# teboli/polyblur

Hardware: AMD Instinct MI355X
Metric: megapixels/sec (n_iter=3, alpha=6, beta=1) (higher is better)
Workload: dtype f32; 1 GPU; batch=1 3840x2160x3 fp32 per GPU, n_iter=3, method=fft (circular), full 25-tap support; mode=resident, images_per_gpu=1, height=2160, width=3840, parallelism=images sharded, no data-path collective

## Files before the change

polyblur_amd/csrc/api.hip:

```cpp
#include <algorithm>
#include <cstdlib>
#include <cstring>

#include "common.h"

int pb_grad_energy(pb_ctx *ctx, const void *gx, const void *gy, float *nM, int P, long HW, int g_dtype = PB_F32);
int pb_halo_apply(pb_ctx *ctx, const void *x, int x_dtype, int x_pitch, long x_plane, const float *y, const void *gx,
                  const void *gy, const void *ox, const float *nM, void *out, int out_dtype, int P, int H, int W,
                  int clamp01, const void *recomb_cur = nullptr, int recomb_cur_dtype = 0, const float *recomb_smooth = nullptr,
                  int g_dtype = PB_F32);
int pb_recombine(pb_ctx *ctx, const float *y, const void *cur, int cur_dtype, const float *smooth, void *out, int out_dtype,
                 long n);
int pb_bilateral5_impl(pb_ctx *ctx, const void *in, int in_dtype, void *out, int out_dtype, int P, int H, int W);
int pb_dt_filter_impl(pb_ctx *ctx, const void *in, const void *joint, int dtype, float *out, int B, int C, int H, int W,
                      float sigma_s, float sigma_r, int num_iterations);
int pb_nc_filter_impl(pb_ctx *ctx, const void *in, int dtype, float *out, int B, int C, int H, int W, float sigma_s,
                      float sigma_r, int num_iterations);
int pb_convert_from_float(pb_ctx *ctx, const float *in, void *out, int dtype, long n);
int pb_u8_layout(pb_ctx *ctx, const unsigned char *in, unsigned char *out, int B, int C, int H, int W, int to_planar);
int pb_convert_to_float(pb_ctx *ctx, const void *in, int dtype, float *out, long n);
int pb_extract_patches_impl(pb_ctx *ctx, const void *img, void *patches, int dtype, int B, int C, int H, int W, int ph, int pw,
                            int step_h, int step_w, int n_j, int pad_top, int pad_left, int first, int count);
int pb_overlap_add_impl(pb_ctx *ctx, const void *patches, void *out, int dtype, int B, int C, int H, int W, int ph, int pw,
                        int step_h, int step_w, int n_i, int n_j, int pad_top, int pad_left, const float *win_y,
// ... 32 lines not shown
    return b.p;
}

static size_t dsize(int dtype) { return dtype == PB_F16 ? 2 : (dtype == PB_U8 ? 1 : 4); }
static int pitch4(int w) { return (w + 3) & ~3; }

static void pb_read_knobs(pb_ctx *ctx) {
    auto geti = [](const char *n, int &v) { if (const char *e = getenv(n)) v = atoi(e); };
    auto getl = [](const char *n, long &v) { if (const char *e = getenv(n)) v = atol(e); };
    if (const char *e = getenv("PB_FFT_BODY")) ctx->fft_wave = (e[0] == 'w' && e[1] == 'g') ? 0 : 1;
#ifdef PB_EXPERIMENTAL
    geti("PB_STRIP", ctx->strip_mode);
#endif
    geti("PB_EST_GRAY_ROWS", ctx->est_gray_rows); geti("PB_EST_LEAN", ctx->est_lean); geti("PB_DT_ROWS_REG", ctx->dt_rows_reg); geti("PB_DT_COLS_STRIP", ctx->dt_cols_strip); geti("PB_DT_COLS_COOP", ctx->dt_cols_coop);
    geti("PB_FFT_EXT_RADIX", ctx->fft_ext_radix); geti("PB_FFT_FIRST", ctx->fft_first); geti("PB_FFT_FIRST_ROWS", ctx->fft_first_rows); geti("PB_COLS_FIXED", ctx->cols_fixed); geti("PB_ROWS_FIXED", ctx->rows_fixed);
    geti("PB_POLY1", ctx->poly_mode);
    geti("PB_POLY_ALWAYS", ctx->poly_always); geti("PB_POLY_PADDED", ctx->poly_padded); geti("PB_TAPER_RING", ctx->taper_ring); geti("PB_ZERO_RING", ctx->zero_ring); getl("PB_ZERO_RING_MIN_PAIRS", ctx->zero_ring_min_pairs);
}

extern "C" {

int pb_version(void) { return PB_VERSION; }

void pb_default_options(pb_options *o) {
    memset(o, 0, sizeof(*o));
    o->n_iter = 1; o->c = 0.352f; o->b = 0.768f; o->alpha = 2.f; o->beta = 3.f;
    o->sigma_r = 0.8f; o->sigma_s = 2.0f; o->q = 0.f; o->n_angles = 6; o->n_interpolated_angles = 30;
    o->remove_halo = 0; o->edgetaping = 0; o->prefilter = PB_PREFILTER_NONE; o->discard_saturation = 0;
    o->boundary = PB_WRAP; o->support = PB_SUPPORT_FULL; o->force_theta_deg = -1.f; o->ker_size = PB_KSIZE;
}

// ... 229 lines not shown
    steps[2] = p;
}

PolySpec poly_spec(pb_ctx *ctx, const ConvPass *steps, float alpha, float beta, bool gaussians) {
    const int mode = pb_poly_spec_mode(ctx, steps);
    if (!mode) {
        if (steps[0].boundary == PB_ZERO && gaussians && ctx->poly_always && pb_poly_three_steps_ok(ctx, steps)) {
            PolySpec ps = no_poly();
            ps.always = 2;
            return ps;
        }
        return no_poly();
    }
    const int always = (mode == 3 && gaussians && ctx->poly_always) ? 1 : 0;
    if (steps[0].boundary != PB_WRAP && !always) return no_poly();
    return PolySpec{mode, alpha / 2 - beta + 2, 3 * beta - alpha - 6, 5 - 3 * beta + alpha / 2, beta, PB_POLY_GAIN, PB_POLY_MIN_AREA, PB_POLY_COST128, always};
}

int run_polynomial(pb_ctx *ctx, const Geometry &g, const void *xsrc, int x_dtype, const float *xpadded,
                   const pb_blur_info *info, float alpha, float beta, int boundary, float *t1, float *t2, void *dst,
                   int dst_dtype, int clamp01) {
    const float a3 = alpha / 2 - beta + 2, a2 = 3 * beta - alpha - 6, a1 = 5 - 3 * beta + alpha / 2;
    if (g.sep1) {
        const float scale[3] = {a3, 1.f, 1.f}, coef[3] = {a2, a1, beta};
        float *tmp[2] = {t1, t2};
        ConvPass p1 = base_pass(g, g.sep1, boundary), p2 = base_pass(g, g.sep2, boundary);
        set_x_virtual(p1, g, xsrc, x_dtype); set_out_padded(p1, g, g.sep_u);
        set_x_virtual(p2, g, xsrc, x_dtype);
        for (int step = 0; step < 3; ++step) {
            if (step < 2) set_out_padded(p2, g, tmp[step]); else set_out_interior(p2, g, dst, dst_dtype);
            p2.scale = scale[step]; p2.coef = coef[step]; p2.clamp01 = step == 2 ? clamp01 : 0;
// ... 858 lines not shown
```

polyblur_amd/csrc/common.h:

```cpp
#pragma once
#include <hip/hip_runtime.h>
#include <hip/hip_fp16.h>

#include <cstdarg>
#include <cstdio>
#include <map>
#include <string>
#include <vector>

#include "../../include/polyblur_hip.h"


struct FftPlan {
    int n = 0;
    int nstage = 0;
    int radix[24];
    int bluestein_m = 0;
    float2 *tw = nullptr;
    float *drev = nullptr;
    float2 *chirp = nullptr;
    float2 *bfilt_rev = nullptr;
    float *dnat = nullptr;
};

struct ScratchBuf {
    void *p = nullptr;
    size_t bytes = 0;
};

struct ProfRec {
    hipEvent_t a, b;
    int tag;
};

struct PolySpec { int on; float a3, a2, a1, b; float gain; int min_area; float cost128; int always; };
inline PolySpec no_poly() { return PolySpec{0, 0.f, 0.f, 0.f, 0.f, 0.f, 0, 0.f, 0}; }
inline bool same_spec(const PolySpec &x, const PolySpec &y) {
    return x.on == y.on && x.always == y.always &&
           (!x.on || (x.a3 == y.a3 && x.a2 == y.a2 && x.a1 == y.a1 && x.b == y.b && (x.cost128 > 0.f) == (y.cost128 > 0.f)));
}

struct pb_fft_sel { int use_fft; int rf; int strip; int poly; int hx; int hy; int pad_[2]; };

struct SpectraSet {
    bool holds(const void *info, int B) const { return owner && owner == info && n == B; }
    bool holds(const void *info, int B, const PolySpec &s) const { return holds(info, B) && same_spec(built, s); }
    void claim(const void *info, int B, const PolySpec &s, int sel_slot, bool by_estimate) {
        owner = info; n = B; built = s; slot_ = sel_slot; est = by_estimate;
    }
    void drop() { owner = nullptr; n = 0; est = false; }
    void drop_if_overlaps(const void *lo, const void *hi) {
        const char *o = static_cast<const char *>(owner);
        if (o && o < static_cast<const char *>(hi) && static_cast<const char *>(lo) < o + sizeof(pb_blur_info) * (size_t)n) drop();
    }
// ... 45 lines not shown
    int zero_ring = 1;
    int taper_ring = 1;
    int poly_padded = 1;
    int est_lean = 1;
    int dt_cols_strip = 1;
    int dt_cols_coop = 1;
    int dt_rows_reg = 1;
    int poly_always = 1;
    int est_gray_rows = 1;
    int fft_ext_radix = 1;
    int fft_first_rows = -1;
    int fft_first = -1;
    int cols_fixed = 1;
    int rows_fixed = 1;
    size_t phase_budget = 0;
    int strip_mode = 0;
};

int pb_fail(pb_ctx *ctx, int code, const char *fmt, ...);

struct ProfScope {
    pb_ctx *ctx;
    int idx = -1;
    ProfScope(pb_ctx *c, int tag) : ctx(c) {
        if (!c->prof_on) return;
        ProfRec r;
        r.tag = tag;
        hipEvent_t *ev[2] = {&r.a, &r.b};
        for (auto e : ev) {
            if (!c->evpool.empty()) { *e = c->evpool.back(); c->evpool.pop_back(); }
// ... 28 lines not shown
    } while (0)

enum { SRC_VIRTUAL = 0,
       SRC_PADDED = 1 };
enum { OUT_INTERIOR = 0,
       OUT_PADDED = 1 };
enum { EPI_HORNER = 0,
       EPI_TAPER = 1 };

constexpr int PB_SEL_SLOTS = 16;
constexpr int PB_KHAT_STRIDE = 128 * 128;
constexpr int PB_POLY128_MIN_T = 56;
constexpr int PB_POLY_MIN_TX = 24, PB_POLY_MIN_TY = 16;
constexpr float PB_POLY_GAIN = 0.7f;
constexpr int PB_POLY_MIN_AREA = 768;
constexpr float PB_POLY_COST128 = 8.0f;


struct ConvPass {
    const void *in;  int in_kind;  int in_dtype;  int in_pitch;  long in_plane;
    const void *x;   int x_kind;   int x_dtype;   int x_pitch;   long x_plane;
    void *out;       int out_kind; int out_dtype; int out_pitch; long out_plane;
    int H, W;
    int pad;
    int C;
    int P;
    const pb_blur_info *info;
    float scale, coef;
    int boundary;
    int epilogue;
// ... 87 lines not shown
```

polyblur_amd/csrc/conv_wave_common.h:

```cpp
#pragma once
#include "conv_fft_common.h"

namespace {

constexpr int WF_ROWS = 32;
constexpr size_t kWfLdsWave = sizeof(float2) * WF_ROWS * FT_P;

static __device__ const float kC64[64] = {
    1.0f, 0.9951847195625305f, 0.9807852506637573f, 0.9569403529167175f, 0.9238795042037964f, 0.8819212913513184f,
    0.8314695954322815f, 0.7730104327201843f, 0.7071067690849304f, 0.6343932747840881f, 0.5555702447891235f,
    0.4713967442512512f, 0.3826834261417389f, 0.290284663438797f, 0.19509032368659973f, 0.0980171412229538f, 0.0f,
    -0.0980171412229538f, -0.19509032368659973f, -0.290284663438797f, -0.3826834261417389f, -0.4713967442512512f,
    -0.5555702447891235f, -0.6343932747840881f, -0.7071067690849304f, -0.7730104327201843f, -0.8314695954322815f,
    -0.8819212913513184f, -0.9238795042037964f, -0.9569403529167175f, -0.9807852506637573f, -0.9951847195625305f, -1.0f,
    -0.9951847195625305f, -0.9807852506637573f, -0.9569403529167175f, -0.9238795042037964f, -0.8819212913513184f,
    -0.8314695954322815f, -0.7730104327201843f, -0.7071067690849304f, -0.6343932747840881f, -0.5555702447891235f,
    -0.4713967442512512f, -0.3826834261417389f, -0.290284663438797f, -0.19509032368659973f, -0.0980171412229538f, 0.0f,
    0.0980171412229538f, 0.19509032368659973f, 0.290284663438797f, 0.3826834261417389f, 0.4713967442512512f,
    0.5555702447891235f, 0.6343932747840881f, 0.7071067690849304f, 0.7730104327201843f, 0.8314695954322815f,
    0.8819212913513184f, 0.9238795042037964f, 0.9569403529167175f, 0.9807852506637573f, 0.9951847195625305f};
static __device__ const float kS64[64] = {
    0.0f, 0.0980171412229538f, 0.19509032368659973f, 0.290284663438797f, 0.3826834261417389f, 0.4713967442512512f,
    0.5555702447891235f, 0.6343932747840881f, 0.7071067690849304f, 0.7730104327201843f, 0.8314695954322815f,
    0.8819212913513184f, 0.9238795042037964f, 0.9569403529167175f, 0.9807852506637573f, 0.9951847195625305f, 1.0f,
// ... 74 lines not shown
#define PB_S(i) fwd_stage1<i>(v);
    PB_EACH8(PB_S)
#undef PB_S
}
__device__ __forceinline__ void fft64_inv_stage1(cf (&v)[64]) {
#define PB_S(i) inv_stage1<i>(v);
    PB_EACH8(PB_S)
#undef PB_S
}
__device__ __forceinline__ void fft64_inv_stage2(cf (&v)[64]) {
#define PB_S(i) inv_stage2<i>(v);
    PB_EACH8(PB_S)
#undef PB_S
}

__device__ __forceinline__ void swap_halves(cf &hi_part, cf &lo_part) {
    typedef unsigned u2 __attribute__((ext_vector_type(2)));
    const u2 x = __builtin_amdgcn_permlane32_swap(__float_as_uint(hi_part.x), __float_as_uint(lo_part.x), false, false);
    const u2 y = __builtin_amdgcn_permlane32_swap(__float_as_uint(hi_part.y), __float_as_uint(lo_part.y), false, false);
    hi_part = (cf){__uint_as_float(x[0]), __uint_as_float(y[0])};
    lo_part = (cf){__uint_as_float(x[1]), __uint_as_float(y[1])};
}

__device__ __forceinline__ void transpose64(cf (&v)[64], float2 *Z, int lane) {
#pragma unroll
    for (int r = 0; r < 32; ++r) swap_halves(v[r], v[32 + r]);
    const float2 *rd = Z + (lane & 31) * FT_P + (lane & 32);
#pragma unroll
    for (int h = 0; h < 2; ++h) {
#pragma unroll
// ... 81 lines not shown
```

polyblur_amd/csrc/conv_wfft.hip:

```cpp

#include <algorithm>
#include <cstdlib>
#include <type_traits>

#include "conv_wave_common.h"

namespace {

struct WGeom { int ow, oh; };
struct WJobs { int pairs_x, njobs, per; float inv_pairs_x; };
__device__ __forceinline__ int div_rcp(int n, float rcp_d) { return (int)(((float)n + 0.5f) * rcp_d); }
__device__ __forceinline__ WJobs jobs_of(const WGeom &g, int hx, int hy) {
    const int Tx = FT_N - 2 * hx, Ty = FT_N - 2 * hy;
    const int tiles_x = div_rcp(g.ow + Tx - 1, __builtin_amdgcn_rcpf((float)Tx)), tiles_y = div_rcp(g.oh + Ty - 1, __builtin_amdgcn_rcpf((float)Ty));
    WJobs j;
    j.pairs_x = (tiles_x + 1) >> 1;
    j.njobs = j.pairs_x * tiles_y;
    j.per = (j.njobs + 7) >> 3;
    j.inv_pairs_x = __builtin_amdgcn_rcpf((float)j.pairs_x);
    return j;
}

#ifdef PB_WF_TRACE
constexpr int kTraceWaves = 8192, kTraceStamps = 14;
__device__ unsigned long long g_wf_trace[kTraceWaves * kTraceStamps];
#define PB_T(i) do { if (tr) { __builtin_amdgcn_sched_barrier(0); tr[i] = __builtin_readcyclecounter(); __builtin_amdgcn_sched_barrier(0); } } while (0)
#define PB_TWAIT() asm volatile("s_waitcnt vmcnt(0) lgkmcnt(0)" ::: "memory")
#define PB_TRT(i) do { if (tr) tr[i] = __builtin_amdgcn_s_memrealtime(); } while (0)
#else
#define PB_T(i)
#define PB_TWAIT()
// ... 425 lines not shown
    typedef std::integral_constant<int, 6> I6; typedef std::integral_constant<int, 7> I7;
    request(I0{}); request(I1{}); request(I2{}); request(I3{});
    fft64_inv_stage2(v);
    PB_T(8);
    finish(I0{}); request(I4{});
    finish(I1{}); request(I5{});
    finish(I2{}); request(I6{});
    finish(I3{}); request(I7{});
    finish(I4{}); finish(I5{}); finish(I6{}); finish(I7{});
    PB_T(9);
    PB_TWAIT();
    PB_T(10);
    PB_TRT(13);
}

template <typename TIn, typename TX, typename TOut>
__device__ __forceinline__ bool pair_is_fast(const ConvPass &a, int ty, int pxi, int hx, int hy) {
    if (sizeof(TIn) < 2 || a.epilogue != EPI_HORNER) return false;
    if (sizeof(TIn) == 2 && (a.in_pitch & 7) != 0) return false;
    const int Tx = FT_N - 2 * hx, Ty = FT_N - 2 * hy;
    const OutRegion rg = out_region(a);
    const int Hp = a.H + 2 * a.pad, Wp = a.W + 2 * a.pad;
    const int oy0 = rg.y_lo + ty * Ty, wy0 = oy0 - hy, wxA = rg.x_lo + 2 * pxi * Tx - hx, wxB = wxA + Tx;
    const int lo = a.in_kind == SRC_VIRTUAL ? a.pad : 0;
    const bool virt = a.x_kind == SRC_VIRTUAL;
    const int oo = a.out_kind == OUT_INTERIOR ? a.pad : 0, xsh = virt ? a.pad : 0;
    const int xw = virt ? a.W : Wp, xh = virt ? a.H : Hp;
    const int oxA = wxA + hx;
    return wy0 >= lo && wy0 + FT_N <= Hp - lo && wxA >= lo && wxB + FT_N <= Wp - lo && oy0 + Ty <= rg.y_hi && oxA + 2 * Tx <= rg.x_hi &&
           oy0 - xsh >= 0 && oxA - xsh >= 0 && oy0 + Ty - xsh <= xh && oxA + 2 * Tx - xsh <= xw &&
// ... 62 lines not shown

template <typename TIn, typename TX, typename TOut, bool ZERO>
__global__ __launch_bounds__(64, 2) void conv_wfft_kernel(const ConvPass a, const WGeom g) {
    extern __shared__ __attribute__((aligned(16))) char zb[];
    const int lane = threadIdx.x & 63;
    unsigned long long *tr = nullptr;
#ifdef PB_WF_TRACE
    if (blockIdx.x < kTraceWaves) tr = g_wf_trace + (long)blockIdx.x * kTraceStamps;
    PB_T(0);
    PB_TRT(12);
#endif
    const int C = a.C, B = a.P / C;
    const int q = (int)(blockIdx.x & 7u);
    int rem = (int)(blockIdx.x >> 3);
    int img = 0, hx = 0, hy = 0;
    bool fold = false;
    if (B == 1) {
        const PB_CONSTANT pb_fft_sel *s0 = as_constant(a.fsel);
        if (!s0->use_fft || s0->poly == 2 || !poly_match(a.poly, s0->poly)) return;
        hx = s0->hx; hy = s0->hy;
        fold = a.poly == 2 && s0->poly != 0;
    } else {
        auto share_of = [&](int i) -> int {
            if (i >= B) return 0;
            const pb_fft_sel s = a.fsel[i];
            if (!s.use_fft || s.poly == 2 || !poly_match(a.poly, s.poly)) return 0;
            return jobs_of(g, s.hx, s.hy).per * C;
        };
        bool work = false;
        int base = 0;
        for (int c0 = 0; c0 < B; c0 += 64) {
            const int n = share_of(c0 + lane), incl = wave_scan(n, lane);
            const unsigned long long m = __ballot(base + incl > rem);
            if (m) {
                const int l = __builtin_ctzll(m);
                img = c0 + l;
                rem -= base + (__builtin_amdgcn_readlane(incl, l) - __builtin_amdgcn_readlane(n, l));
                work = true;
                break;
            }
            base += __builtin_amdgcn_readlane(incl, 63);
        }
        if (!work) return;
        img = __builtin_amdgcn_readfirstlane(img); rem = __builtin_amdgcn_readfirstlane(rem);
        hx = as_constant(a.fsel + img)->hx; hy = as_constant(a.fsel + img)->hy;
        fold = a.poly == 2 && as_constant(a.fsel + img)->poly != 0;
    }
    const WJobs j = jobs_of(g, hx, hy);
    const int pl = __builtin_amdgcn_readfirstlane(div_rcp(rem, __builtin_amdgcn_rcpf((float)j.per)));
    if (pl >= C) return;
    const int pair = q * j.per + (rem - pl * j.per);
    if (pair >= j.njobs) return;
    const int ty = __builtin_amdgcn_readfirstlane(div_rcp(pair, j.inv_pairs_x)), pxi = pair - ty * j.pairs_x;
    const int plane = img * C + pl;
    const float *kp = a.khat + (long)img * PB_KHAT_STRIDE;
    const pb_blur_info *info = a.info + img;
    if (a.ring && !ring_live(a, ty, pxi, hx, hy)) return;
    const ConvPass af = fold_pass(a, fold);
    if (taper_is_copy(af, ty, pxi, hx, hy)) { copy_pair<TX, TOut>(af, plane, ty, pxi, hx, hy); return; }
    if (pair_is_fast<TIn, TX, TOut>(af, ty, pxi, hx, hy)) wave_pair<1, TIn, TX, TOut, ZERO>(af, info, plane, ty, pxi, hx, hy, zb, kp, tr);
    else if (pair_is_gen<TIn, TX, TOut>(af, pxi, hx)) wave_pair<2, TIn, TX, TOut, ZERO>(af, info, plane, ty, pxi, hx, hy, zb, kp, tr);
    else wave_pair<0, TIn, TX, TOut, ZERO>(af, info, plane, ty, pxi, hx, hy, zb, kp, tr);
}

bool wfft_geometry(const ConvPass &p, bool poly2, float min_area, WGeom &g, long &per_max) {
    g.oh = (p.out_kind == OUT_INTERIOR) ? p.H : p.H + 2 * p.pad;
    g.ow = (p.out_kind == OUT_INTERIOR) ? p.W : p.W + 2 * p.pad;
    per_max = 0;
    for (int hx = 4; hx <= 28; hx += 4) {
        for (int hy = 2; hy <= 30; hy += 2) {
            const int tx = FT_N - 2 * hx, ty = FT_N - 2 * hy;
            const bool three = hx <= 12 && hy <= 12;
            const bool one = poly2 && tx >= PB_POLY_MIN_TX && ty >= PB_POLY_MIN_TY && (float)(tx * ty) >= min_area;
            if (!three && !one) continue;
            const long nj = (long)(((g.ow + tx - 1) / tx + 1) / 2) * ((g.oh + ty - 1) / ty);
            if (nj > (1L << 20)) return false;
            per_max = std::max(per_max, (nj + 7) / 8);
        }
    }
    const long total = 8 * per_max * p.P;
    return total > 0 && total <= (1L << 23);
}

template <typename TIn, typename TX, typename TOut>
int launch_wfft_typed(pb_ctx *ctx, const ConvPass &p, const WGeom &g, long groups) {
    if (p.boundary == PB_ZERO)
        hipLaunchKernelGGL((conv_wfft_kernel<TIn, TX, TOut, true>), dim3((unsigned)groups), dim3(64), kWfLdsWave, ctx->stream, p, g);
    else
        hipLaunchKernelGGL((conv_wfft_kernel<TIn, TX, TOut, false>), dim3((unsigned)groups), dim3(64), kWfLdsWave, ctx->stream, p, g);
    PB_LAUNCH_CHECK();
    return PB_OK;
}

// ... 1 lines not shown

#ifdef PB_WF_TRACE
extern "C" int pb_debug_wf_trace_clear(void) {
    void *p = nullptr;
    if (hipGetSymbolAddress(&p, HIP_SYMBOL(g_wf_trace)) != hipSuccess) return -1;
    return (int)hipMemset(p, 0, sizeof(unsigned long long) * kTraceStamps * kTraceWaves);
}
extern "C" int pb_debug_wf_trace(unsigned long long *host, int n_waves) {
    if (n_waves > kTraceWaves) n_waves = kTraceWaves;
    return (int)hipMemcpyFromSymbol(host, HIP_SYMBOL(g_wf_trace), sizeof(unsigned long long) * kTraceStamps * n_waves);
}
#endif

bool pb_conv_wfft_feasible(const ConvPass &p, bool poly2) {
    WGeom g; long per_max = 0;
    return wfft_geometry(p, poly2, (float)PB_POLY_MIN_AREA, g, per_max);
}

bool pb_conv_wfft_types(const ConvPass &p) {
    switch (p.in_dtype * 9 + p.x_dtype * 3 + p.out_dtype) {
        case 0: case 1: case 3: case 4: case 12: case 13: case 24: case 26: case 6: case 8: case 2: return true;
        default: return false;
    }
}

int pb_launch_conv_wfft(pb_ctx *ctx, const ConvPass &p) {
    if (!pb_conv_wfft_types(p)) return PB_ERR_UNSUPPORTED;
    const bool poly2 = p.poly != 0 && pb_spec_of_spectra(ctx, p.khat).on >= 2;
    const float min_area = (float)PB_POLY_MIN_AREA;
    WGeom g;
    long per_max = 0;
    if (!wfft_geometry(p, poly2, min_area, g, per_max)) {
        if (poly2) return pb_fail(ctx, PB_ERR_UNSUPPORTED, "conv pass: too many windows for the tile-spectrum body");
        return PB_ERR_UNSUPPORTED;
    }
    long groups = 8L * per_max * p.P;
    if (ctx->known_sel) {
        const int B = p.P / p.C;
        long per_sum = 0, jobs = 0;
        for (int b = 0; b < B && b < (int)ctx->known_sel->size(); ++b) {
            const pb_fft_sel &e = (*ctx->known_sel)[(size_t)b];
            const bool takes = e.use_fft && e.poly != 2 && (p.poly == 2 || (e.poly != 0) == (p.poly != 0));
            if (!takes) continue;
            const int tx = FT_N - 2 * e.hx, ty = FT_N - 2 * e.hy;
            const long nj = (long)(((g.ow + tx - 1) / tx + 1) / 2) * ((g.oh + ty - 1) / ty);
            per_sum += (nj + 7) / 8; jobs += nj * p.C;
        }
        if (!jobs) return PB_OK;
        groups = 8L * per_sum * p.C;
    }
    ProfScope prof(ctx, PB_PROF_CONV_FFT);
    switch (p.in_dtype * 9 + p.x_dtype * 3 + p.out_dtype) {
        case 0: return launch_wfft_typed<float, float, float>(ctx, p, g, groups);
        case 1: return launch_wfft_typed<float, float, __half>(ctx, p, g, groups);
        case 3: return launch_wfft_typed<float, __half, float>(ctx, p, g, groups);
        case 4: return launch_wfft_typed<float, __half, __half>(ctx, p, g, groups);
        case 12: return launch_wfft_typed<__half, __half, float>(ctx, p, g, groups);
        case 13: return launch_wfft_typed<__half, __half, __half>(ctx, p, g, groups);
        case 24: return launch_wfft_typed<unsigned char, unsigned char, float>(ctx, p, g, groups);
        case 26: return launch_wfft_typed<unsigned char, unsigned char, unsigned char>(ctx, p, g, groups);
// ... 7 lines not shown
```

polyblur_amd/csrc/khat.h:

```cpp
#pragma once
#include "common.h"
#ifndef PB_PT
#define PB_PT(i)
#endif

namespace {

constexpr int KH_FT_N = 64, KH_THREADS = 256;
static __device__ const double kCos64[64] = {
    1, 0.99518472667219693, 0.98078528040323043, 0.95694033573220882,
    0.92387953251128674, 0.88192126434835505, 0.83146961230254524, 0.77301045336273699,
    0.70710678118654757, 0.63439328416364549, 0.55557023301960229, 0.47139673682599781,
    0.38268343236508984, 0.29028467725446233, 0.19509032201612833, 0.09801714032956077,
    0, -0.098017140329560645, -0.19509032201612819, -0.29028467725446216,
    -0.38268343236508973, -0.4713967368259977, -0.55557023301960196, -0.63439328416364538,
    -0.70710678118654746, -0.77301045336273699, -0.83146961230254535, -0.88192126434835494,
    -0.92387953251128674, -0.95694033573220882, -0.98078528040323043, -0.99518472667219682,
    -1, -0.99518472667219693, -0.98078528040323043, -0.95694033573220894,
    -0.92387953251128685, -0.88192126434835505, -0.83146961230254546, -0.7730104533627371,
    -0.70710678118654768, -0.63439328416364593, -0.55557023301960218, -0.47139673682599786,
    -0.38268343236509034, -0.29028467725446244, -0.19509032201612866, -0.098017140329560451,
    0, 0.09801714032956009, 0.1950903220161283, 0.29028467725446205,
    0.38268343236509, 0.47139673682599759, 0.55557023301960184, 0.6343932841636456,
    0.70710678118654735, 0.77301045336273666, 0.83146961230254524, 0.88192126434835483,
// ... 149 lines not shown
__device__ __forceinline__ void khat_body(const pb_blur_info *info, float *out, pb_fft_sel *sel, int min_phases, int slice,
                                          const PolySpec ps = no_poly(), const RecLds *rl = nullptr, bool lean = false) {
    constexpr int NR = PB_KRAD + 1, PXS = KH_FT_N / SL;
    __shared__ double c8[128], s8[128];
    constexpr int K1 = PB_KSIZE, K2 = 2 * PB_KSIZE - 1, K3 = 3 * PB_KSIZE - 2;
    __shared__ double2 G[NR * PXS];
    __shared__ double cs[KH_FT_N], sn[KH_FT_N];
    __shared__ float sk[PB_KSIZE * PB_KSIZE];
    __shared__ float s_m[2][K1], s_mp[2][3 * K1 - 2], s_m2[2][K2 + 2 * (K1 - 1)], s_m3[2][K3];
    __shared__ int s_h[4];
    const int tid = threadIdx.x, lane = tid & 63, wave = tid >> 6;
    const int nph = rl ? rl->nph : info->nphase[0] + info->nphase[1] + info->nphase[2];
    const int R = rl ? rl->radius : info->radius;
    const int separable = rl ? rl->separable : info->separable;
    if (tid < KH_FT_N) { cs[tid] = kCos64[tid]; sn[tid] = kSin64[tid]; }
    if (ps.on == 3 && tid >= 64 && tid < 192) { c8[tid - 64] = kCos128[tid - 64]; s8[tid - 64] = kSin128[tid - 64]; }
    bool sym = true;
    const float *skp = lean ? rl->taps : sk;
    if (!lean)
    for (int i = tid; i < PB_KSIZE * PB_KSIZE; i += KH_THREADS) {
        const int u = i / PB_KSIZE - PB_KRAD, v = i % PB_KSIZE - PB_KRAD;
        const bool in = abs(u) <= R && abs(v) <= R;
        const float k = rl ? rl->taps[i] : info->kernel[i];
        const float km = rl ? rl->taps[PB_KSIZE * PB_KSIZE - 1 - i] : info->kernel[PB_KSIZE * PB_KSIZE - 1 - i];
        sk[i] = in ? k : 0.f;
        sym = sym && (!in || k == km);
    }
    constexpr int PD = K1 - 1;
    if (tid < 2 * (K1 + 2 * PD)) s_mp[tid / (K1 + 2 * PD)][tid % (K1 + 2 * PD)] = 0.f;
    if (tid < 2 * (K2 + 2 * PD)) s_m2[tid / (K2 + 2 * PD)][tid % (K2 + 2 * PD)] = 0.f;
    PB_PT(20);
// ... 44 lines not shown
                    if (i >= 2 * PB_KRAD && i < 2 * PB_KRAD + K1) v += c1 * s_m[ax][i - 2 * PB_KRAD];
                    return v;
                }, 3 * PB_KRAD, KH_HALO_TOL, lane);
        } else {
            r = 3 * PB_KRAD;
        }
        if (lane == 0) s_h[wave] = r;
    }
    __syncthreads();
    PB_PT(26);
    const int hxk = max(4, (s_h[0] + 3) & ~3), hyk = max(2, (s_h[1] + 1) & ~1);
    const int hxp = max(4, (s_h[2] + 3) & ~3), hyp = max(2, (s_h[3] + 1) & ~1);
    const int Rh = max(4, (max(s_h[0], s_h[1]) + 3) & ~3);
    const bool dense = symm && separable == 0;
    const bool use3 = ps.always == 2 ? symm : (dense && nph >= min_phases + (R <= 4 && min_phases > 0 ? 8 : 0));
    bool poly = false, poly128 = false;
    if (ps.on == 1) poly = symm && Rh <= 4 && max(hxp, hyp) <= 12;
    if (ps.on >= 2 && symm) {
        const int txp = KH_FT_N - 2 * hxp, typ = KH_FT_N - 2 * hyp;
        const float ak = (float)((KH_FT_N - 2 * hxk) * (KH_FT_N - 2 * hyk));
        const float c3 = ps.always == 1 ? INFINITY : (use3 ? 3.f / (ps.gain * ak) : 1.f / (float)ps.min_area);
        float c64 = INFINITY, c128 = INFINITY;
        if (txp >= PB_POLY_MIN_TX && typ >= PB_POLY_MIN_TY && txp * typ >= ps.min_area) c64 = 1.f / (float)(txp * typ);
        const int tx8 = 2 * KH_FT_N - 2 * hxp, ty8 = 2 * KH_FT_N - 2 * hyp;
        if (ps.on == 3 && ps.cost128 > 0.f && tx8 >= PB_POLY128_MIN_T && ty8 >= PB_POLY128_MIN_T) c128 = ps.cost128 / (float)(tx8 * ty8);
        poly128 = c128 < c64 && c128 < c3;
        poly = poly128 || c64 <= c3;
    }
    const bool use = poly || use3;
    if (tid == 0 && slice == 0) {
        sel->use_fft = use ? 1 : 0;
        sel->rf = poly ? (ps.on == 1 ? 12 : (vouched_wrongly ? -1 : 0)) : Rh;
        sel->hx = poly ? hxp : hxk; sel->hy = poly ? hyp : hyk;
        if (!lean) sel->strip = (separable != 0 && R > 8) ? 1 : 0;
        sel->poly = poly128 ? 2 : (poly ? 1 : 0);
        sel->pad_[0] = 0;
        if (!lean) sel->pad_[1] = 0;
    }
    PB_PT(23);
    if (poly128) { khat128_body<SL>(skp, out, slice, ps, c8, s8); PB_PT(22); return; }
    if (!use) return;
    const int px0 = slice * PXS;
    if (tid < NR * PXS) {
        const int u = tid / PXS + PB_KRAD, px = px0 + tid % PXS, fx = (px >> 3) + 8 * (px & 7);
        double ar = 0.0, ai = 0.0;
#pragma unroll 5
        for (int v = 0; v < PB_KSIZE; ++v) {
            const int m = (fx * (v - PB_KRAD)) & 63;
            const double k = (double)skp[u * PB_KSIZE + v];
            ar += k * cs[m]; ai += k * sn[m];
        }
        G[tid] = make_double2(ar, ai);
    }
    __syncthreads();
    PB_PT(21);
    for (int idx = tid; idx < PXS * KH_FT_N; idx += KH_THREADS) {
        const int pxl = idx >> 6, py = idx & 63, fy = (py >> 3) + 8 * (py & 7);
        double ar = 0.5 * G[pxl].x;
#pragma unroll 4
        for (int u = 1; u < NR; ++u) {
            const int m = (fy * u) & 63;
            const double2 g = G[u * PXS + pxl];
            ar += g.x * cs[m] - g.y * sn[m];
        }
        double v = 2.0 * ar;
        if (poly) v = (((double)ps.a3 * v + (double)ps.a2) * v + (double)ps.a1) * v + (double)ps.b;
        out[(px0 + pxl) * KH_FT_N + py] = (float)(v * (1.0 / 4096.0));
    }
    PB_PT(22);
}
// ... 3 lines not shown
```

Measured before the change: 16830 MP/s.

## Add tall 64x128 real-FFT tile path for polynomial wrap deconvolution

Adds a 'tall' tile mode that packs two real 64-row halves into one complex 64-point FFT along columns, giving 64x128 tiles with a real split/merge step and centre-symmetric spectrum multiply. The khat kernel gains a cost model that picks this mode when it beats the 64x64 and 128 paths, and emits the half-spectrum with a Nyquist row. It aims to cut the halo overhead and FFT work per output pixel. The price is more selection logic and extra register pressure in the new wave body. It is enabled by default through poly_tall=1.

New measurement: 17400 MP/s, median of 6. 1.03x the previous value.

```diff
diff --git a/polyblur_amd/csrc/api.hip b/polyblur_amd/csrc/api.hip
--- a/polyblur_amd/csrc/api.hip
+++ b/polyblur_amd/csrc/api.hip
@@ -70,7 +70,7 @@
 #endif
     geti("PB_EST_GRAY_ROWS", ctx->est_gray_rows); geti("PB_EST_LEAN", ctx->est_lean); geti("PB_DT_ROWS_REG", ctx->dt_rows_reg); geti("PB_DT_COLS_STRIP", ctx->dt_cols_strip); geti("PB_DT_COLS_COOP", ctx->dt_cols_coop);
     geti("PB_FFT_EXT_RADIX", ctx->fft_ext_radix); geti("PB_FFT_FIRST", ctx->fft_first); geti("PB_FFT_FIRST_ROWS", ctx->fft_first_rows); geti("PB_COLS_FIXED", ctx->cols_fixed); geti("PB_ROWS_FIXED", ctx->rows_fixed);
-    geti("PB_POLY1", ctx->poly_mode);
+    geti("PB_POLY1", ctx->poly_mode); geti("PB_POLY_TALL", ctx->poly_tall);
     geti("PB_POLY_ALWAYS", ctx->poly_always); geti("PB_POLY_PADDED", ctx->poly_padded); geti("PB_TAPER_RING", ctx->taper_ring); geti("PB_ZERO_RING", ctx->zero_ring); getl("PB_ZERO_RING_MIN_PAIRS", ctx->zero_ring_min_pairs);
 }
 
@@ -330,7 +330,12 @@
     }
     const int always = (mode == 3 && gaussians && ctx->poly_always) ? 1 : 0;
     if (steps[0].boundary != PB_WRAP && !always) return no_poly();
-    return PolySpec{mode, alpha / 2 - beta + 2, 3 * beta - alpha - 6, 5 - 3 * beta + alpha / 2, beta, PB_POLY_GAIN, PB_POLY_MIN_AREA, PB_POLY_COST128, always};
+    const ConvPass &f = steps[0], &l = steps[2];
+    const bool tall_ok = mode >= 2 && f.boundary == PB_WRAP && f.in_dtype == PB_F32 && f.x_dtype == PB_F32 && l.out_dtype == PB_F32 &&
+                         f.in_kind == SRC_VIRTUAL && f.epilogue == EPI_HORNER && f.H >= 128;
+    const int tall = tall_ok ? std::min(std::max(ctx->poly_tall, 0), 2) : 0;
+    return PolySpec{mode, alpha / 2 - beta + 2, 3 * beta - alpha - 6, 5 - 3 * beta + alpha / 2, beta, PB_POLY_GAIN, PB_POLY_MIN_AREA, PB_POLY_COST128, always,
+                    tall, PB_POLY_COST_TALL};
 }
 
 int run_polynomial(pb_ctx *ctx, const Geometry &g, const void *xsrc, int x_dtype, const float *xpadded,
diff --git a/polyblur_amd/csrc/common.h b/polyblur_amd/csrc/common.h
--- a/polyblur_amd/csrc/common.h
+++ b/polyblur_amd/csrc/common.h
@@ -33,11 +33,11 @@
     int tag;
 };
 
-struct PolySpec { int on; float a3, a2, a1, b; float gain; int min_area; float cost128; int always; };
-inline PolySpec no_poly() { return PolySpec{0, 0.f, 0.f, 0.f, 0.f, 0.f, 0, 0.f, 0}; }
+struct PolySpec { int on; float a3, a2, a1, b; float gain; int min_area; float cost128; int always; int tall; float cost_tall; };
+inline PolySpec no_poly() { return PolySpec{0, 0.f, 0.f, 0.f, 0.f, 0.f, 0, 0.f, 0, 0, 0.f}; }
 inline bool same_spec(const PolySpec &x, const PolySpec &y) {
     return x.on == y.on && x.always == y.always &&
-           (!x.on || (x.a3 == y.a3 && x.a2 == y.a2 && x.a1 == y.a1 && x.b == y.b && (x.cost128 > 0.f) == (y.cost128 > 0.f)));
+           (!x.on || (x.a3 == y.a3 && x.a2 == y.a2 && x.a1 == y.a1 && x.b == y.b && (x.cost128 > 0.f) == (y.cost128 > 0.f) && x.tall == y.tall));
 }
 
 struct pb_fft_sel { int use_fft; int rf; int strip; int poly; int hx; int hy; int pad_[2]; };
@@ -113,6 +113,7 @@
     int cols_fixed = 1;
     int rows_fixed = 1;
     size_t phase_budget = 0;
+    int poly_tall = 1;
     int strip_mode = 0;
 };
 
@@ -171,6 +172,10 @@
 constexpr int PB_POLY_MIN_TX = 24, PB_POLY_MIN_TY = 16;
 constexpr float PB_POLY_GAIN = 0.7f;
 constexpr int PB_POLY_MIN_AREA = 768;
+constexpr int PB_TALL_MIN_AREA = 2 * PB_POLY_MIN_AREA;
+constexpr int PB_TALL_MAX_HY = 36;
+constexpr float PB_POLY_COST_TALL = 1.22f;
+constexpr float PB_POLY_COST128_BARE = 6.5f;
 constexpr float PB_POLY_COST128 = 8.0f;
 
 
diff --git a/polyblur_amd/csrc/conv_wave_common.h b/polyblur_amd/csrc/conv_wave_common.h
--- a/polyblur_amd/csrc/conv_wave_common.h
+++ b/polyblur_amd/csrc/conv_wave_common.h
@@ -112,6 +112,95 @@
 #undef PB_S
 }
 
+static __device__ const float kCr128[33] = {
+    1.0f, 0.9987954497337341f, 0.9951847195625305f, 0.9891765117645264f, 0.9807852506637573f, 0.9700312614440918f,
+    0.9569403529167175f, 0.9415440559387207f, 0.9238795042037964f, 0.903989315032959f, 0.8819212913513184f,
+    0.8577286005020142f, 0.8314695954322815f, 0.803207516670227f, 0.7730104327201843f, 0.7409511208534241f,
+    0.7071067690849304f, 0.6715589761734009f, 0.6343932747840881f, 0.5956993103027344f, 0.5555702447891235f,
+    0.5141027569770813f, 0.4713967442512512f, 0.4275550842285156f, 0.3826834261417389f, 0.3368898630142212f,
+    0.290284663438797f, 0.24298018217086792f, 0.19509032368659973f, 0.1467304676771164f, 0.0980171412229538f,
+    0.049067676067352295f, 0.0f};
+static __device__ const float kSr128[33] = {
+    0.0f, 0.049067676067352295f, 0.0980171412229538f, 0.1467304676771164f, 0.19509032368659973f, 0.24298018217086792f,
+    0.290284663438797f, 0.3368898630142212f, 0.3826834261417389f, 0.4275550842285156f, 0.4713967442512512f,
+    0.5141027569770813f, 0.5555702447891235f, 0.5956993103027344f, 0.6343932747840881f, 0.6715589761734009f,
+    0.7071067690849304f, 0.7409511208534241f, 0.7730104327201843f, 0.803207516670227f, 0.8314695954322815f,
+    0.8577286005020142f, 0.8819212913513184f, 0.903989315032959f, 0.9238795042037964f, 0.9415440559387207f,
+    0.9569403529167175f, 0.9700312614440918f, 0.9807852506637573f, 0.9891765117645264f, 0.9951847195625305f,
+    0.9987954497337341f, 1.0f};
+constexpr int reg_of_freq(int k) { return 8 * (k & 7) + (k >> 3); }
+template <int K> __device__ __forceinline__ void real_split_pair(cf (&v)[64]) {
+    constexpr int ra = reg_of_freq(K), rb = reg_of_freq(64 - K);
+    const float c = kCr128[K], s = kSr128[K];
+    const cf A = v[ra], B = v[rb];
+    const float ex = A.x + B.x, ey = A.y - B.y, dx = A.x - B.x, dy = A.y + B.y;
+    v[ra] = (cf){fmaf(c, dy, fmaf(-s, dx, ex)), fmaf(-c, dx, fmaf(-s, dy, ey))};
+    v[rb] = (cf){fmaf(-c, dy, fmaf(s, dx, ex)), fmaf(-c, dx, fmaf(-s, dy, -ey))};
+}
+template <int K> __device__ __forceinline__ void real_merge_pair(cf (&v)[64]) {
+    constexpr int ra = reg_of_freq(K), rb = reg_of_freq(64 - K);
+    const float c = kCr128[K], s = kSr128[K];
+    const cf P = v[ra], B = v[rb];
+    const float ex = P.x + B.x, ey = P.y - B.y, dx = P.x - B.x, dy = P.y + B.y;
+    v[ra] = (cf){fmaf(-c, dy, fmaf(-s, dx, ex)), fmaf(c, dx, fmaf(-s, dy, ey))};
+    v[rb] = (cf){fmaf(c, dy, fmaf(s, dx, ex)), fmaf(c, dx, fmaf(-s, dy, -ey))};
+}
+#define PB_EACH31(F) F(1) F(2) F(3) F(4) F(5) F(6) F(7) F(8) F(9) F(10) F(11) F(12) F(13) F(14) F(15) F(16) F(17) F(18) F(19) F(20) \
+    F(21) F(22) F(23) F(24) F(25) F(26) F(27) F(28) F(29) F(30) F(31)
+__device__ __forceinline__ void real_split(cf (&v)[64]) {
+#define PB_S(i) real_split_pair<i>(v);
+    PB_EACH31(PB_S)
+#undef PB_S
+    v[reg_of_freq(32)] = (cf){2.f * v[reg_of_freq(32)].x, -2.f * v[reg_of_freq(32)].y};
+    v[0] = (cf){2.f * (v[0].x + v[0].y), 2.f * (v[0].x - v[0].y)};
+}
+__device__ __forceinline__ void real_merge(cf (&v)[64]) {
+#define PB_S(i) real_merge_pair<i>(v);
+    PB_EACH31(PB_S)
+#undef PB_S
+    v[reg_of_freq(32)] = (cf){2.f * v[reg_of_freq(32)].x, -2.f * v[reg_of_freq(32)].y};
+    v[0] = (cf){v[0].x + v[0].y, v[0].x - v[0].y};
+}
+template <int K1> __device__ __forceinline__ void centre_finish(cf (&v)[64], cf (&b)[8]) {
+    ibf8(b);
+#pragma unroll
+    for (int n2 = 0; n2 < 8; ++n2) {
+        const int m = (n2 * K1) & 63;
+        v[8 * K1 + n2] = m ? cmul_conj_s(b[n2], (cf){kC64[m], -kS64[m]}) : b[n2];
+    }
+}
+template <int K1> __device__ __forceinline__ void centre_self_real(cf (&v)[64], const float (&kh)[8], const PB_CONSTANT float *hd, float f) {
+    static_assert(K1 == 0 || K1 == 4, "groups 0 and 4 meet themselves");
+    cf b[8], o[8];
+#pragma unroll
+    for (int n2 = 0; n2 < 8; ++n2) b[n2] = v[8 * K1 + n2];
+    bf8(b);
+#pragma unroll
+    for (int k2 = 0; k2 < 8; ++k2) {
+        const int p = K1 == 0 ? ((8 - k2) & 7) : 7 - k2;
+        const float g = f * hd[8 * K1 + k2];
+        o[k2] = (cf){fmaf(g, b[p].x, b[k2].x * kh[k2]), fmaf(-g, b[p].y, b[k2].y * kh[k2])};
+    }
+    centre_finish<K1>(v, o);
+}
+template <int KA, int KB> __device__ __forceinline__ void centre_pair_real(cf (&v)[64], const float (&kha)[8], const float (&khb)[8],
+                                                                           const PB_CONSTANT float *hd, float f) {
+    static_assert(KA + KB == 8 && KA != KB, "groups K1 and 8 - K1");
+    cf b[8], c[8], ob[8], oc[8];
+#pragma unroll
+    for (int n2 = 0; n2 < 8; ++n2) { b[n2] = v[8 * KA + n2]; c[n2] = v[8 * KB + n2]; }
+    bf8(b);
+    bf8(c);
+#pragma unroll
+    for (int k2 = 0; k2 < 8; ++k2) {
+        const float ga = f * hd[8 * KA + k2], gb = f * hd[8 * KB + k2];
+        ob[k2] = (cf){fmaf(ga, c[7 - k2].x, b[k2].x * kha[k2]), fmaf(-ga, c[7 - k2].y, b[k2].y * kha[k2])};
+        oc[k2] = (cf){fmaf(gb, b[7 - k2].x, c[k2].x * khb[k2]), fmaf(-gb, b[7 - k2].y, c[k2].y * khb[k2])};
+    }
+    centre_finish<KA>(v, ob);
+    centre_finish<KB>(v, oc);
+}
+
 __device__ __forceinline__ void swap_halves(cf &hi_part, cf &lo_part) {
     typedef unsigned u2 __attribute__((ext_vector_type(2)));
     const u2 x = __builtin_amdgcn_permlane32_swap(__float_as_uint(hi_part.x), __float_as_uint(lo_part.x), false, false);
diff --git a/polyblur_amd/csrc/conv_wfft.hip b/polyblur_amd/csrc/conv_wfft.hip
--- a/polyblur_amd/csrc/conv_wfft.hip
+++ b/polyblur_amd/csrc/conv_wfft.hip
@@ -10,11 +10,11 @@
 struct WGeom { int ow, oh; };
 struct WJobs { int pairs_x, njobs, per; float inv_pairs_x; };
 __device__ __forceinline__ int div_rcp(int n, float rcp_d) { return (int)(((float)n + 0.5f) * rcp_d); }
-__device__ __forceinline__ WJobs jobs_of(const WGeom &g, int hx, int hy) {
-    const int Tx = FT_N - 2 * hx, Ty = FT_N - 2 * hy;
+__device__ __forceinline__ WJobs jobs_of(const WGeom &g, int hx, int hy, bool tall) {
+    const int Tx = FT_N - 2 * hx, Ty = (tall ? 2 * FT_N : FT_N) - 2 * hy;
     const int tiles_x = div_rcp(g.ow + Tx - 1, __builtin_amdgcn_rcpf((float)Tx)), tiles_y = div_rcp(g.oh + Ty - 1, __builtin_amdgcn_rcpf((float)Ty));
     WJobs j;
-    j.pairs_x = (tiles_x + 1) >> 1;
+    j.pairs_x = tall ? tiles_x : (tiles_x + 1) >> 1;
     j.njobs = j.pairs_x * tiles_y;
     j.per = (j.njobs + 7) >> 3;
     j.inv_pairs_x = __builtin_amdgcn_rcpf((float)j.pairs_x);
@@ -470,6 +470,187 @@
     PB_TRT(13);
 }
 
+__device__ __forceinline__ void wave_tall(const ConvPass &a, int plane, int ty, int txi, int hx, int hy, char *zb, const float *kp) {
+    constexpr int TN = 2 * FT_N;
+    const int Tx = FT_N - 2 * hx, Ty = TN - 2 * hy;
+    float2 *Z = reinterpret_cast<float2 *>(zb);
+    float *Zf = reinterpret_cast<float *>(zb);
+    const OutRegion rg = out_region(a);
+    const int oy0 = rg.y_lo + ty * Ty, ox0 = rg.x_lo + txi * Tx;
+    const int wx = ox0 - hx, wy0 = oy0 - hy;
+    const int wrap_r = TN - hy;
+    const int lane = threadIdx.x & 63;
+    const float *ipl = static_cast<const float *>(a.in) + (long)plane * a.in_plane;
+    float *opl = static_cast<float *>(a.out) + (long)plane * a.out_plane;
+    const int Hp = a.H + 2 * a.pad, Wp = a.W + 2 * a.pad;
+    cf v[64];
+    {
+        const brsrc rin = plane_rsrc(ipl, a.in_plane);
+        const int lo = a.in_kind == SRC_VIRTUAL ? a.pad : 0;
+        const int pitchb = a.in_pitch * 4;
+        lds_char *zl = lds_ptr(zb);
+        const unsigned la = lds_addr(zb) + (unsigned)lane * 4u;
+        auto pick = [&](int k, int buf) {
+#pragma unroll
+            for (int j = 0; j < 8; ++j) {
+                const unsigned ad = la + (unsigned)(buf * 8192 + j * 1024);
+                asm volatile("ds_read2_b32 %0, %1 offset1:64" : "=v"(v[8 * j + 2 * k]) : "v"(ad));
+                asm volatile("ds_read2_b32 %0, %1 offset0:128 offset1:192" : "=v"(v[8 * j + 2 * k + 1]) : "v"(ad));
+            }
+            asm volatile("s_waitcnt lgkmcnt(0)" : "+v"(v[2 * k]), "+v"(v[2 * k + 1]), "+v"(v[8 + 2 * k]), "+v"(v[9 + 2 * k]), "+v"(v[16 + 2 * k]),
+                         "+v"(v[17 + 2 * k]), "+v"(v[24 + 2 * k]), "+v"(v[25 + 2 * k]), "+v"(v[32 + 2 * k]), "+v"(v[33 + 2 * k]), "+v"(v[40 + 2 * k]),
+                         "+v"(v[41 + 2 * k]), "+v"(v[48 + 2 * k]), "+v"(v[49 + 2 * k]), "+v"(v[56 + 2 * k]), "+v"(v[57 + 2 * k]) :: "memory");
+        };
+        if (wy0 >= lo && wy0 + TN <= Hp - lo && wx >= lo && wx + FT_N <= Wp - lo && ((a.in_pitch | (wx - lo)) & 3) == 0) {
+            auto rowoff = [&](int r) -> int { return (oy0 - lo + r - (r >= wrap_r ? TN : 0)) * pitchb; };
+            const unsigned colb = (unsigned)((wx - lo + 4 * (lane & 15)) * 4);
+            const unsigned vo = (unsigned)((lane >> 4) * pitchb) + colb;
+            const unsigned vos = (unsigned)((lane < 32 ? TN - 2 + (lane >> 4) : (lane >> 4) - 2) * pitchb) + colb;
+            auto request = [&](int k, int buf) {
+#pragma unroll
+                for (int j = 0; j < 8; ++j) {
+                    const int r0 = 16 * j + 4 * k;
+                    const bool straddle = r0 + 2 == wrap_r;
+                    dma16<0>(rin, zl + buf * 8192 + j * 1024, straddle ? vos : vo, rowoff(straddle ? r0 + 2 : r0));
+                }
+            };
+            request(0, 0); request(1, 1);
+            asm volatile("s_waitcnt vmcnt(8)" ::: "memory");
+            pick(0, 0);
+            request(2, 0);
+            asm volatile("s_waitcnt vmcnt(8)" ::: "memory");
+            pick(1, 1);
+            request(3, 1);
+            asm volatile("s_waitcnt vmcnt(8)" ::: "memory");
+            pick(2, 0);
+            wait_vm0();
+            pick(3, 1);
+        } else {
+            const unsigned gcol = (unsigned)map_axis(wx + lane, a.W, a.in_kind, PB_WRAP, a.pad) * 4u;
+            const int base = __builtin_amdgcn_readfirstlane(wrap_idx(oy0, Hp));
+            const bool virt_in = a.in_kind == SRC_VIRTUAL;
+            auto gather = [&](int k, int buf) {
+#pragma unroll
+                for (int i = 0; i < 32; ++i) {
+                    const int r = 16 * (i >> 2) + 4 * k + (i & 3);
+                    int pr = base + r - (r >= wrap_r ? TN : 0);
+                    pr += pr < 0 ? Hp : 0;
+                    pr -= pr >= Hp ? Hp : 0;
+                    const int so = (virt_in ? min(max(pr - a.pad, 0), a.H - 1) : pr) * pitchb;
+                    dma4<0>(rin, zl + buf * 8192 + i * 256, gcol, so);
+                }
+            };
+            gather(0, 0); gather(1, 1);
+            asm volatile("s_waitcnt vmcnt(32)" ::: "memory");
+            pick(0, 0);
+            gather(2, 0);
+            asm volatile("s_waitcnt vmcnt(32)" ::: "memory");
+            pick(1, 1);
+            gather(3, 1);
+            asm volatile("s_waitcnt vmcnt(32)" ::: "memory");
+            pick(2, 0);
+            wait_vm0();
+            pick(3, 1);
+        }
+    }
+    fft64_fwd(v);
+    real_split(v);
+    transpose64(v, Z, lane);
+    {
+        const brsrc rk = plane_rsrc(kp, (long)FT_N * FT_N);
+        const PB_CONSTANT float *hd = as_constant(kp + FT_N * FT_N);
+        const float f0 = lane == 0 ? 1.f : 0.f;
+        float kh[4][8];
+        auto khload = [&](int slot, int grp) {
+#pragma unroll
+            for (int k2 = 0; k2 < 8; ++k2) kh[slot][k2] = BufIO<float>::ld(rk, (unsigned)lane * 4u, (8 * grp + k2) * (FT_N * 4));
+        };
+        khload(0, 0); khload(1, 1); khload(2, 7); khload(3, 2);
+        __builtin_amdgcn_sched_barrier(0);
+        fft64_fwd_stage1(v);
+        centre_self_real<0>(v, kh[0], hd, f0); khload(0, 6); __builtin_amdgcn_sched_barrier(0);
+        centre_pair_real<1, 7>(v, kh[1], kh[2], hd, f0); khload(1, 3); khload(2, 5); __builtin_amdgcn_sched_barrier(0);
+        centre_pair_real<2, 6>(v, kh[3], kh[0], hd, f0); khload(3, 4); __builtin_amdgcn_sched_barrier(0);
+        centre_pair_real<3, 5>(v, kh[1], kh[2], hd, f0);
+        centre_self_real<4>(v, kh[3], hd, f0);
+    }
+    fft64_inv_stage1(v);
+    transpose64(v, Z, lane);
+    real_merge(v);
+    fft64_inv_stage2(v);
+    fft64_inv_stage1(v);
+
+    const int oo = a.out_kind == OUT_INTERIOR ? a.pad : 0;
+    const int opitchb = a.out_pitch * 4;
+    const brsrc ro = plane_rsrc(opl, a.out_plane);
+    const bool colin = lane >= hx && lane < FT_N - hx;
+    const float sc = a.scale;
+    const float clo = a.clamp01 ? 0.f : -INFINITY, chi = a.clamp01 ? 1.f : INFINITY;
+    const int tyr = min(Ty, rg.y_hi - oy0);
+    if (((a.out_pitch | (ox0 - oo)) & 3) == 0 && ox0 + Tx <= rg.x_hi) {
+        const int C = Tx >> 2;
+        const float invC = __builtin_amdgcn_rcpf((float)C);
+        int rlk[4], chk[4];
+#pragma unroll
+        for (int k = 0; k < 4; ++k) {
+            const int e = 64 * k + lane;
+            rlk[k] = div_small(e, invC); chk[k] = e - rlk[k] * C;
+        }
+        const int oso = (oy0 - oo) * opitchb + (ox0 - oo) * 4;
+        auto round = [&](auto qc) {
+            constexpr int q = decltype(qc)::value;
+            const int left = tyr - 16 * q;
+            f4v acc[4];
+#pragma unroll
+            for (int k = 0; k < 4; ++k) acc[k] = *reinterpret_cast<const f4v *>(Zf + (16 * (q & 3) + min(rlk[k], 15)) * FT_N + 4 * chk[k]);
+#pragma unroll
+            for (int k = 0; k < 4; ++k) {
+                f4v o;
+                o.x = __builtin_amdgcn_fmed3f(sc * acc[k].x, clo, chi); o.y = __builtin_amdgcn_fmed3f(sc * acc[k].y, clo, chi);
+                o.z = __builtin_amdgcn_fmed3f(sc * acc[k].z, clo, chi); o.w = __builtin_amdgcn_fmed3f(sc * acc[k].w, clo, chi);
+                const bool ok = rlk[k] < min(left, 16);
+                st_b128(ro, ok ? (unsigned)(rlk[k] * opitchb + chk[k] * 16) : kNoAccess, oso + 16 * q * opitchb, o);
+            }
+        };
+        float *zt = Zf + (lane - hx);
+        auto put_half = [&](auto hc) {
+            constexpr int h = decltype(hc)::value;
+            if (colin) {
+#pragma unroll
+                for (int i = 0; i < 32; ++i) { zt[2 * i * FT_N] = v[32 * h + i].x; zt[(2 * i + 1) * FT_N] = v[32 * h + i].y; }
+            }
+        };
+        typedef std::integral_constant<int, 0> Q0; typedef std::integral_constant<int, 1> Q1; typedef std::integral_constant<int, 2> Q2;
+        typedef std::integral_constant<int, 3> Q3; typedef std::integral_constant<int, 4> Q4; typedef std::integral_constant<int, 5> Q5;
+        typedef std::integral_constant<int, 6> Q6; typedef std::integral_constant<int, 7> Q7;
+        put_half(Q0{});
+        wave_lds_fence();
+        round(Q0{}); round(Q1{}); round(Q2{}); round(Q3{});
+        wave_lds_fence();
+        put_half(Q1{});
+        wave_lds_fence();
+        if (tyr > 64) {
+            round(Q4{});
+            if (tyr > 80) {
+                round(Q5{});
+                if (tyr > 96) {
+                    round(Q6{});
+                    if (tyr > 112) round(Q7{});
+                }
+            }
+        }
+        return;
+    }
+    const bool okc = colin && wx + lane < rg.x_hi;
+    const unsigned ooff = okc ? (unsigned)(wx + lane - oo) * 4u : kNoAccess;
+#pragma unroll
+    for (int n = 0; n < 64; ++n) {
+        const int so = (oy0 + 2 * n - oo) * opitchb;
+        BufIO<float>::st(ro, 2 * n < tyr ? ooff : kNoAccess, so, __builtin_amdgcn_fmed3f(sc * v[n].x, clo, chi));
+        BufIO<float>::st(ro, 2 * n + 1 < tyr ? ooff : kNoAccess, so + opitchb, __builtin_amdgcn_fmed3f(sc * v[n].y, clo, chi));
+    }
+}
+
 template <typename TIn, typename TX, typename TOut>
 __device__ __forceinline__ bool pair_is_fast(const ConvPass &a, int ty, int pxi, int hx, int hy) {
     if (sizeof(TIn) < 2 || a.epilogue != EPI_HORNER) return false;
@@ -562,18 +743,20 @@
     const int q = (int)(blockIdx.x & 7u);
     int rem = (int)(blockIdx.x >> 3);
     int img = 0, hx = 0, hy = 0;
-    bool fold = false;
+    bool fold = false, tall = false;
+    constexpr bool kTall = std::is_same<TIn, float>::value && std::is_same<TX, float>::value && std::is_same<TOut, float>::value && !ZERO;
     if (B == 1) {
         const PB_CONSTANT pb_fft_sel *s0 = as_constant(a.fsel);
         if (!s0->use_fft || s0->poly == 2 || !poly_match(a.poly, s0->poly)) return;
         hx = s0->hx; hy = s0->hy;
         fold = a.poly == 2 && s0->poly != 0;
+        tall = kTall && s0->poly == 1 && s0->pad_[0] != 0;
     } else {
         auto share_of = [&](int i) -> int {
             if (i >= B) return 0;
             const pb_fft_sel s = a.fsel[i];
             if (!s.use_fft || s.poly == 2 || !poly_match(a.poly, s.poly)) return 0;
-            return jobs_of(g, s.hx, s.hy).per * C;
+            return jobs_of(g, s.hx, s.hy, kTall && s.poly == 1 && s.pad_[0] != 0).per * C;
         };
         bool work = false;
         int base = 0;
@@ -593,8 +776,9 @@
         img = __builtin_amdgcn_readfirstlane(img); rem = __builtin_amdgcn_readfirstlane(rem);
         hx = as_constant(a.fsel + img)->hx; hy = as_constant(a.fsel + img)->hy;
         fold = a.poly == 2 && as_constant(a.fsel + img)->poly != 0;
-    }
-    const WJobs j = jobs_of(g, hx, hy);
+        tall = kTall && as_constant(a.fsel + img)->poly == 1 && as_constant(a.fsel + img)->pad_[0] != 0;
+    }
+    const WJobs j = jobs_of(g, hx, hy, tall);
     const int pl = __builtin_amdgcn_readfirstlane(div_rcp(rem, __builtin_amdgcn_rcpf((float)j.per)));
     if (pl >= C) return;
     const int pair = q * j.per + (rem - pl * j.per);
@@ -605,13 +789,16 @@
     const pb_blur_info *info = a.info + img;
     if (a.ring && !ring_live(a, ty, pxi, hx, hy)) return;
     const ConvPass af = fold_pass(a, fold);
+    if constexpr (kTall) {
+        if (tall) { wave_tall(af, plane, ty, pxi, hx, hy, zb, kp); return; }
+    }
     if (taper_is_copy(af, ty, pxi, hx, hy)) { copy_pair<TX, TOut>(af, plane, ty, pxi, hx, hy); return; }
     if (pair_is_fast<TIn, TX, TOut>(af, ty, pxi, hx, hy)) wave_pair<1, TIn, TX, TOut, ZERO>(af, info, plane, ty, pxi, hx, hy, zb, kp, tr);
     else if (pair_is_gen<TIn, TX, TOut>(af, pxi, hx)) wave_pair<2, TIn, TX, TOut, ZERO>(af, info, plane, ty, pxi, hx, hy, zb, kp, tr);
     else wave_pair<0, TIn, TX, TOut, ZERO>(af, info, plane, ty, pxi, hx, hy, zb, kp, tr);
 }
 
-bool wfft_geometry(const ConvPass &p, bool poly2, float min_area, WGeom &g, long &per_max) {
+bool wfft_geometry(const ConvPass &p, bool poly2, bool tall, float min_area, WGeom &g, long &per_max) {
     g.oh = (p.out_kind == OUT_INTERIOR) ? p.H : p.H + 2 * p.pad;
     g.ow = (p.out_kind == OUT_INTERIOR) ? p.W : p.W + 2 * p.pad;
     per_max = 0;
@@ -625,6 +812,13 @@
             if (nj > (1L << 20)) return false;
             per_max = std::max(per_max, (nj + 7) / 8);
         }
+        for (int hy = 2; poly2 && tall && hy <= PB_TALL_MAX_HY; hy += 2) {
+            const int tx = FT_N - 2 * hx, tyt = 2 * FT_N - 2 * hy;
+            if (tx < PB_POLY_MIN_TX || tx * tyt < PB_TALL_MIN_AREA) continue;
+            const long nj = (long)((g.ow + tx - 1) / tx) * ((g.oh + tyt - 1) / tyt);
+            if (nj > (1L << 20)) return false;
+            per_max = std::max(per_max, (nj + 7) / 8);
+        }
     }
     const long total = 8 * per_max * p.P;
     return total > 0 && total <= (1L << 23);
@@ -656,7 +850,7 @@
 
 bool pb_conv_wfft_feasible(const ConvPass &p, bool poly2) {
     WGeom g; long per_max = 0;
-    return wfft_geometry(p, poly2, (float)PB_POLY_MIN_AREA, g, per_max);
+    return wfft_geometry(p, poly2, poly2 && p.boundary == PB_WRAP, (float)PB_POLY_MIN_AREA, g, per_max);
 }
 
 bool pb_conv_wfft_types(const ConvPass &p) {
@@ -672,7 +866,8 @@
     const float min_area = (float)PB_POLY_MIN_AREA;
     WGeom g;
     long per_max = 0;
-    if (!wfft_geometry(p, poly2, min_area, g, per_max)) {
+    const bool tall = poly2 && pb_spec_of_spectra(ctx, p.khat).tall != 0;
+    if (!wfft_geometry(p, poly2, tall, min_area, g, per_max)) {
         if (poly2) return pb_fail(ctx, PB_ERR_UNSUPPORTED, "conv pass: too many windows for the tile-spectrum body");
         return PB_ERR_UNSUPPORTED;
     }
@@ -684,8 +879,10 @@
             const pb_fft_sel &e = (*ctx->known_sel)[(size_t)b];
             const bool takes = e.use_fft && e.poly != 2 && (p.poly == 2 || (e.poly != 0) == (p.poly != 0));
             if (!takes) continue;
-            const int tx = FT_N - 2 * e.hx, ty = FT_N - 2 * e.hy;
-            const long nj = (long)(((g.ow + tx - 1) / tx + 1) / 2) * ((g.oh + ty - 1) / ty);
+            const bool et = tall && e.poly == 1 && e.pad_[0] != 0;
+            const int tx = FT_N - 2 * e.hx, ty = (et ? 2 * FT_N : FT_N) - 2 * e.hy;
+            const long tiles_x = (g.ow + tx - 1) / tx;
+            const long nj = (et ? tiles_x : (tiles_x + 1) / 2) * ((g.oh + ty - 1) / ty);
             per_sum += (nj + 7) / 8; jobs += nj * p.C;
         }
         if (!jobs) return PB_OK;
diff --git a/polyblur_amd/csrc/khat.h b/polyblur_amd/csrc/khat.h
--- a/polyblur_amd/csrc/khat.h
+++ b/polyblur_amd/csrc/khat.h
@@ -187,7 +187,7 @@
     const int R = rl ? rl->radius : info->radius;
     const int separable = rl ? rl->separable : info->separable;
     if (tid < KH_FT_N) { cs[tid] = kCos64[tid]; sn[tid] = kSin64[tid]; }
-    if (ps.on == 3 && tid >= 64 && tid < 192) { c8[tid - 64] = kCos128[tid - 64]; s8[tid - 64] = kSin128[tid - 64]; }
+    if ((ps.on == 3 || ps.tall) && tid >= 64 && tid < 192) { c8[tid - 64] = kCos128[tid - 64]; s8[tid - 64] = kSin128[tid - 64]; }
     bool sym = true;
     const float *skp = lean ? rl->taps : sk;
     if (!lean)
@@ -262,7 +262,7 @@
     const int Rh = max(4, (max(s_h[0], s_h[1]) + 3) & ~3);
     const bool dense = symm && separable == 0;
     const bool use3 = ps.always == 2 ? symm : (dense && nph >= min_phases + (R <= 4 && min_phases > 0 ? 8 : 0));
-    bool poly = false, poly128 = false;
+    bool poly = false, poly128 = false, tall = false;
     if (ps.on == 1) poly = symm && Rh <= 4 && max(hxp, hyp) <= 12;
     if (ps.on >= 2 && symm) {
         const int txp = KH_FT_N - 2 * hxp, typ = KH_FT_N - 2 * hyp;
@@ -272,8 +272,12 @@
         if (txp >= PB_POLY_MIN_TX && typ >= PB_POLY_MIN_TY && txp * typ >= ps.min_area) c64 = 1.f / (float)(txp * typ);
         const int tx8 = 2 * KH_FT_N - 2 * hxp, ty8 = 2 * KH_FT_N - 2 * hyp;
         if (ps.on == 3 && ps.cost128 > 0.f && tx8 >= PB_POLY128_MIN_T && ty8 >= PB_POLY128_MIN_T) c128 = ps.cost128 / (float)(tx8 * ty8);
-        poly128 = c128 < c64 && c128 < c3;
-        poly = poly128 || c64 <= c3;
+        float ctall = INFINITY;
+        const bool tall_ok = ps.tall != 0 && txp >= PB_POLY_MIN_TX && hyp <= PB_TALL_MAX_HY && txp * (2 * KH_FT_N - 2 * hyp) >= PB_TALL_MIN_AREA;
+        if (tall_ok) ctall = 2.f * ps.cost_tall / (float)(txp * (2 * KH_FT_N - 2 * hyp));
+        tall = tall_ok && (ps.tall == 2 || (ctall < c64 && ctall < c128 * (PB_POLY_COST128_BARE / PB_POLY_COST128) && ctall < c3));
+        poly128 = !tall && c128 < c64 && c128 < c3;
+        poly = poly128 || tall || c64 <= c3;
     }
     const bool use = poly || use3;
     if (tid == 0 && slice == 0) {
@@ -282,7 +286,7 @@
         sel->hx = poly ? hxp : hxk; sel->hy = poly ? hyp : hyk;
         if (!lean) sel->strip = (separable != 0 && R > 8) ? 1 : 0;
         sel->poly = poly128 ? 2 : (poly ? 1 : 0);
-        sel->pad_[0] = 0;
+        sel->pad_[0] = tall ? 1 : 0;
         if (!lean) sel->pad_[1] = 0;
     }
     PB_PT(23);
@@ -302,6 +306,31 @@
     }
     __syncthreads();
     PB_PT(21);
+    if (tall) {
+        for (int idx = tid; idx < PXS * KH_FT_N; idx += KH_THREADS) {
+            const int pxl = idx >> 6, py = idx & 63, fy = (py >> 3) + 8 * (py & 7);
+            auto at = [&](int f) {
+                double ar = 0.5 * G[pxl].x;
+#pragma unroll 4
+                for (int u = 1; u < NR; ++u) {
+                    const int m = (f * u) & 127;
+                    const double2 g = G[u * PXS + pxl];
+                    ar += g.x * c8[m] - g.y * s8[m];
+                }
+                const double v = 2.0 * ar;
+                return ((((double)ps.a3 * v + (double)ps.a2) * v + (double)ps.a1) * v + (double)ps.b) * (1.0 / 16384.0);
+            };
+            if (py) {
+                out[(px0 + pxl) * KH_FT_N + py] = (float)at(fy);
+            } else {
+                const double h0 = at(0), h64 = at(64);
+                out[(px0 + pxl) * KH_FT_N] = (float)(0.5 * (h0 + h64));
+                out[KH_FT_N * KH_FT_N + px0 + pxl] = (float)(0.5 * (h0 - h64));
+            }
+        }
+        PB_PT(22);
+        return;
+    }
     for (int idx = tid; idx < PXS * KH_FT_N; idx += KH_THREADS) {
         const int pxl = idx >> 6, py = idx & 63, fy = (py >> 3) + 8 * (py & 7);
         double ar = 0.5 * G[pxl].x;
```
